# jzbontar/mc-cnn

Measured on AMD Instinct MI355X. Metric: Mega-pixel-disparities/sec (cost-vol+CBCA+SGM) + end-to-end disp ms/pair, higher is better.
Workload: dtype f32; 1 GPU; KITTI 2012 fast, 370x1226 disp_max=228; H=370, W=1226, disp_max=228, feature_channels=64, params=kitti_fast, parallelism=one pair per GPU

## Files before the change

### mc-cnn_amd/csrc/api.hip

```cpp
#include "launchers.h"

using namespace mc;

#define MC_REQUIRE_DIRECTION(name, direction) MC_REQUIRE((direction) == -1 || (direction) == 1, name ": direction must be -1 or 1")

struct PlanArea { size_t off, bytes; };
static PlanArea plan_area(int D, int H, int W) { return {align_up(cbca_scratch_bytes(H, W), 256), cbca_plan_bytes(D, H, W)}; }

extern "C" {

int mc_version(void) { return MC_ABI_VERSION; }
const char *mc_last_error(void) { return last_error(); }

int mc_fill_nan(float *p, int64_t n, void *stream)
{
	MC_REQUIRE(p || n == 0, "mc_fill_nan: null pointer");
	MC_REQUIRE(n >= 0, "mc_fill_nan: negative size");
	return fill_nan(p, n, as_stream(stream));
}

int mc_stereo_join(const float *featL, const float *featR, float *volL, float *volR, int C, int D, int H, int W, void *stream)
{
	MC_REQUIRE(featL && featR && volL && volR, "mc_stereo_join: null pointer");
	MC_REQUIRE(dims_ok(D, H, W) && C >= 1, "mc_stereo_join: bad dims C=%d D=%d H=%d W=%d", C, D, H, W);
// ... 240 lines not shown

size_t mc_sgm2_tmp_bytes(int H, int W, int D)
{
	(void)D;
	if (H < 1 || W < 1) return 0;
	return sgm_maps_bytes(H, W);
}

int mc_sgm2(const float *x0, const float *x1, const float *in_hwd, float *out_hwd, void *tmp, size_t tmp_bytes, int H, int W,
            int D, float pi1, float pi2, float tau_so, float alpha1, float sgm_q1, float sgm_q2, int direction, void *stream)
{
	MC_REQUIRE(x0 && x1 && in_hwd && out_hwd && tmp, "mc_sgm2: null pointer");
	MC_REQUIRE(dims_ok(D, H, W), "mc_sgm2: bad dims");
	MC_REQUIRE(D <= MC_SGM_MAX_D, "mc_sgm2: D=%d exceeds %d", D, MC_SGM_MAX_D);
	MC_REQUIRE_DIRECTION("mc_sgm2", direction);
	MC_REQUIRE(tmp_bytes >= sgm_maps_bytes(H, W), "mc_sgm2: tmp holds %zu bytes, needs %zu", tmp_bytes, sgm_maps_bytes(H, W));
	MC_REQUIRE(in_hwd != out_hwd, "mc_sgm2: input and output must differ");
	hipStream_t st = as_stream(stream);
	int rc = sgm_prep(x0, x1, tmp, H, W, tau_so, st);
	if (rc) return rc;
	const float *Cv[2] = {in_hwd, in_hwd};
	float *outv[2] = {out_hwd, out_hwd};
	const int dirv[2] = {direction, direction};
	return sgm_sweeps(Cv, outv, nullptr, nullptr, dirv, 1, H, W, D, D, tmp, pi1, pi2, alpha1, sgm_q1, sgm_q2, false, 0u, false, st);
}

int mc_dhw_to_hwd(const float *in, float *out, int D, int H, int W, void *stream)
{
	MC_REQUIRE(in && out && in != out, "mc_dhw_to_hwd: bad pointers");
	MC_REQUIRE(dims_ok(D, H, W), "mc_dhw_to_hwd: bad dims");
	return transpose(in, out, D, (int64_t)H * W, (int64_t)H * W, D, 1.0f, as_stream(stream));
}

int mc_hwd_to_dhw(const float *in, float *out, int D, int H, int W, float scale_, void *stream)
{
	MC_REQUIRE(in && out && in != out, "mc_hwd_to_dhw: bad pointers");
	MC_REQUIRE(dims_ok(D, H, W), "mc_hwd_to_dhw: bad dims");
	return transpose(in, out, (int64_t)H * W, D, D, (int64_t)H * W, scale_, as_stream(stream));
}

int mc_scale(const float *in, float *out, int64_t n, float s, void *stream)
{
	MC_REQUIRE((in && out) || n == 0, "mc_scale: null pointer");
	MC_REQUIRE(n >= 0, "mc_scale: negative size");
	return scale(in, out, n, s, as_stream(stream));
}

int mc_argmin(const float *vol, float *disp, int D, int H, int W, void *stream)
{
	MC_REQUIRE(vol && disp, "mc_argmin: null pointer");
	MC_REQUIRE(dims_ok(D, H, W), "mc_argmin: bad dims");
	return argmin_dhw(vol, disp, D, H, W, 0, as_stream(stream));
}

int mc_spatial_argmin(const float *vol, float *out, int D, int H, int W, void *stream)
{
	MC_REQUIRE(vol && out, "mc_spatial_argmin: null pointer");
	MC_REQUIRE(dims_ok(D, H, W), "mc_spatial_argmin: bad dims");
	return argmin_dhw(vol, out, D, H, W, 1, as_stream(stream));
}

int mc_outlier_detection(const float *d0, const float *d1, float *outlier, int H, int W, int disp_max, void *stream)
{
	MC_REQUIRE(d0 && d1 && outlier, "mc_outlier_detection: null pointer");
	MC_REQUIRE(dims_ok(1, H, W) && disp_max >= 0, "mc_outlier_detection: bad dims");
	return outlier_detection(d0, d1, outlier, H, W, disp_max, as_stream(stream));
}

int mc_interpolate_occlusion(const float *d0, const float *outlier, float *out, int H, int W, void *stream)
{
	MC_REQUIRE(d0 && outlier && out && out != d0, "mc_interpolate_occlusion: bad pointers");
	MC_REQUIRE(dims_ok(1, H, W), "mc_interpolate_occlusion: bad dims");
	return interpolate_occlusion(d0, outlier, out, H, W, as_stream(stream));
}

int mc_interpolate_mismatch(const float *d0, const float *outlier, float *out, int H, int W, void *stream)
{
	MC_REQUIRE(d0 && outlier && out && out != d0, "mc_interpolate_mismatch: bad pointers");
	MC_REQUIRE(dims_ok(1, H, W), "mc_interpolate_mismatch: bad dims");
	return interpolate_mismatch(d0, outlier, out, H, W, as_stream(stream));
}

int mc_subpixel_enchancement(const float *d0, const float *vol, float *out, int D, int H, int W, void *stream)
{
	MC_REQUIRE(d0 && vol && out, "mc_subpixel_enchancement: null pointer");
	MC_REQUIRE(dims_ok(D, H, W), "mc_subpixel_enchancement: bad dims");
	return subpixel(d0, vol, out, D, H, W, (int64_t)H * W, 1, as_stream(stream));
}

int mc_median2d(const float *img, float *out, int H, int W, int kernel_size, void *stream)
{
	MC_REQUIRE(img && out && img != out, "mc_median2d: bad pointers");
	MC_REQUIRE(dims_ok(1, H, W), "mc_median2d: bad dims");
	MC_REQUIRE(kernel_size % 2 == 1 && kernel_size >= 1 && kernel_size <= 11,
	           "mc_median2d: kernel_size must be odd and <= 11 (adcensus.cu:1601-1602)");
	return median2d(img, out, H, W, kernel_size, as_stream(stream));
}

int mc_mean2d(const float *img, const float *kernel, float *out, int H, int W, int ks, float alpha2, void *stream)
{
	MC_REQUIRE(img && kernel && out && img != out, "mc_mean2d: bad pointers");
	MC_REQUIRE(dims_ok(1, H, W), "mc_mean2d: bad dims");
	MC_REQUIRE(ks % 2 == 1 && ks >= 1, "mc_mean2d: kernel size must be odd (adcensus.cu:1269)");
	return mean2d(img, kernel, out, H, W, ks, alpha2, as_stream(stream));
}

int mc_gaussian_host(double sigma, float *host_kernel, int capacity)
{
	MC_REQUIRE(sigma > 0, "mc_gaussian_host: sigma must be > 0");
	const int ks = gaussian_ks(sigma);
	if (host_kernel) {
		MC_REQUIRE(capacity >= ks * ks, "mc_gaussian_host: capacity %d < %d", capacity, ks * ks);
		gaussian_fill(sigma, host_kernel);
	}
	return ks;
}

int mc_normalize_forward(const float *in, float *norm, float *out, int N, int C, int H, int W, void *stream)
{
	MC_REQUIRE(in && out, "mc_normalize_forward: null pointer");
	MC_REQUIRE(N >= 1 && C >= 1 && dims_ok(1, H, W), "mc_normalize_forward: bad dims");
	return normalize_forward(in, norm, out, N, C, H, W, as_stream(stream));
}

size_t mc_predict_workspace_bytes(const mc_params *p, int C, int D, int H, int W)
{
	(void)C;
	if (!p || !dims_ok(D, H, W) || !(p->blur_sigma > 0)) return 0;
	return make_plan(p, D, H, W).total;
}

int mc_predict(const mc_params *p, const float *x0, const float *x1, const float *featL, const float *featR, int C,
               const float *rawL, const float *rawR, int D, int H, int W, void *workspace, size_t workspace_bytes,
               float *volL_out, float *volR_out, float *dispL0_out, float *dispR0_out, float *disp_out, void *stream)
{
	StageTimer tm;
	return predict_impl(p, x0, x1, featL, featR, C, rawL, rawR, D, H, W, workspace, workspace_bytes, volL_out, volR_out,
	                    dispL0_out, dispR0_out, disp_out, as_stream(stream), tm);
}

int mc_predict_timed(const mc_params *p, const float *x0, const float *x1, const float *featL, const float *featR, int C,
                     const float *rawL, const float *rawR, int D, int H, int W, void *workspace, size_t workspace_bytes,
                     float *disp_out, void *stream, float *stage_ms)
{
	StageTimer tm;
	tm.on = stage_ms != nullptr;
	tm.st = as_stream(stream);
	const int rc = predict_impl(p, x0, x1, featL, featR, C, rawL, rawR, D, H, W, workspace, workspace_bytes, nullptr, nullptr,
	                            nullptr, nullptr, disp_out, tm.st, tm);
	if (stage_ms) tm.collect(stage_ms);
	return rc;
}

}
```

### mc-cnn_amd/csrc/launchers.h

```cpp
#pragma once
#include "cbca_common.h"

#include <vector>

namespace mc {

int fill_nan(float *p, int64_t n, hipStream_t st);
int scale(const float *in, float *out, int64_t n, float s, hipStream_t st);
int transpose(const float *in, float *out, int64_t R, int64_t Cn, int64_t ldin, int64_t ldout, float s, hipStream_t st, int nt = -1);
int fix_border(float *vol, int D, int H, int W, int n, int direction, hipStream_t st);
int argmin_dhw(const float *vol, float *out, int D, int H, int W, int base1, hipStream_t st);
int outlier_detection(const float *d0, const float *d1, float *outlier, int H, int W, int disp_max, hipStream_t st);
constexpr int MC_MIS_MASK_MAX_PIXELS = 524288;
int interpolate_occlusion(const float *d0, const float *outlier, float *out, int H, int W, hipStream_t st, unsigned *mask = nullptr);
int interpolate_mismatch(const float *d0, const float *outlier, float *out, int H, int W, hipStream_t st, const unsigned *mask = nullptr);
int subpixel(const float *d0, const float *vol, float *out, int D, int H, int W, int64_t sd, int64_t sp, hipStream_t st);
int median2d(const float *img, float *out, int H, int W, int k, hipStream_t st);
int mean2d(const float *img, const float *kernel, float *out, int H, int W, int ks, float alpha2, hipStream_t st);
int normalize_forward(const float *in, float *norm, float *out, int N, int C, int H, int W, hipStream_t st);

int stereo_join_dhw(const float *fL, const float *fR, float *volL, float *volR, int C, int D, int H, int W, hipStream_t st);
int stereo_join_hwd(const float *fL, const float *fR, float *volL, float *volR, int C, int D, int ds, int H, int W, int n, hipStream_t st);
int ad_tiled(const float *x0, const float *x1, float *vol, int D, int H, int W, int direction, hipStream_t st);
size_t census_scratch_bytes(int Cimg, int H, int W);
int census_sig(const float *x0, const float *x1, float *vol, void *scratch, int Cimg, int D, int H, int W, int direction, hipStream_t st);

int cross(const float *img, float *arms, int H, int W, int L1, float tau1, hipStream_t st);
int cbca(const float *x0c, const float *x1c, const float *vin, float *vout, int D, int H, int W, int direction, hipStream_t st);
size_t cbca_scratch_bytes(int H, int W);
int cbca_pack(const float *x0c, const float *x1c, void *scratch, int H, int W, hipStream_t st);
int cbca_if_overflow(const float *x0c, const float *x1c, const void *packed, const float *vin, float *vout, int D, int H, int W, int direction, hipStream_t st);
int cbca_strips(const void *packed, const float *vin, float *vout, int D, int H, int W, int direction, int route,
                hipStream_t st, const CbcaCfg &cfg = CbcaCfg());
bool packed_dims_ok(int H, int W);
int cbca_by_arms(const void *packed, const float *vin, float *vout, int D, int H, int W, int direction, int max_arm, hipStream_t st,
                 const CbcaCfg &cfg = CbcaCfg());

size_t cbca_plan_bytes(int D, int H, int W);
int cbca_tiles(const void *packed, const float *vin, float *vout, int D, int H, int W, int direction, int arm_class, int route,
               hipStream_t st, const CbcaCfg &cfg = CbcaCfg());

int cbca_lean_rows(int D, int H, int W, int rb, bool two_pass);
size_t cbca_lean2x_bytes(int D, int H, int W);
bool cbca_lean_fits(int D, int H, int W, size_t plan_bytes, bool two_pass = false, int rb = 0);
int cbca_classify(const void *packed, void *plan, size_t plan_bytes, int D, int H, int W, int direction, int route, int rb, int cap_limit,
                  hipStream_t st, bool two_pass = false, float cost_limit = 0);
int cbca_lean2x(const void *packed, const void *plan, size_t plan_bytes, const float *vin, float *vout, int D, int H, int W, int direction,
                int route, hipStream_t st, const CbcaCfg &cfg);
int cbca_lean(const void *packed, const void *plan, size_t plan_bytes, const float *vin, float *vout, int D, int H, int W, int direction,
              int route, hipStream_t st, const CbcaCfg &cfg);

size_t conv3x3_workspace_bytes(int Cin, int Cout);
int conv3x3(const float *in, const float *w, const float *bias, float *out, int N, int Cin, int Cout, int H, int W, int relu, void *workspace, hipStream_t st);

size_t fc_workspace_bytes(int C, int n_hidden, int H, int W);
int fc_stack(const float *featL, const float *featR, int C, int H, int W, int D, const float *const *weights,
             const float *const *biases, int n_layers, float *volL, float *volR, void *workspace, hipStream_t st);

size_t sgm_maps_bytes(int H, int W);
int sgm_prep(const float *x0, const float *x1, void *maps, int H, int W, float tau_so, hipStream_t st);
int sgm_contract_violations(const float *vol, int H, int W, int D, unsigned *count, hipStream_t st);
int sgm_sweeps(const float *const C[2], float *const out[2], float *const out2[2], float *const disp[2],
               const int direction[2], int nvol, int H, int W, int D, int ds, const void *maps, float pi1, float pi2,
               float alpha1, float q1, float q2, bool fused, unsigned drop_final, bool tri, hipStream_t st);

static inline int gaussian_ks(double sigma) { return 2 * (int)ceil(sigma * 3) + 1; }
void gaussian_fill(double sigma, float *k);

struct Plan {
	int Dp;
	size_t cplan_bytes;
	size_t total;
	void *maps, *packed;
	float *x0c, *x1c, *img[6], *gk;
	float *bufA[2], *bufB[2], *bufC[2];
	void *cplan[2];
};
Plan make_plan(const mc_params *p, int D, int H, int W, void *base = nullptr);

struct StageTimer {
	bool on = false;
	hipStream_t st;
	std::vector<hipEvent_t> ev;
	std::vector<int> tag;
	void mark(int stage);
	void collect(float out[MC_N_STAGES]);
};
int predict_impl(const mc_params *p, const float *x0, const float *x1, const float *featL, const float *featR, int C,
                 const float *rawL, const float *rawR, int D, int H, int W, void *workspace, size_t workspace_bytes,
                 float *volL_out, float *volR_out, float *dispL0_out, float *dispR0_out, float *disp_out, hipStream_t st,
                 StageTimer &tm);

}
```

### mc-cnn_amd/csrc/predict.hip

```cpp
#include "launchers.h"

#include <map>
#include <mutex>
#include <utility>

namespace mc {

void gaussian_fill(double sigma, float *k)
{
	const int ks = gaussian_ks(sigma), kr = ks / 2;
	for (int i = 1; i <= ks; ++i) {
		for (int j = 1; j <= ks; ++j) {
			const double y = (i - 1) - kr;
			const double x = (j - 1) - kr;
			k[(size_t)(i - 1) * ks + (j - 1)] = (float)exp(-(x * x + y * y) / (2 * sigma * sigma));
		}
	}
}
static int gaussian_cached(double sigma, const float *&out)
{
	static std::mutex mu;
	static std::map<std::pair<int, double>, const float *> cache;
	int dev = 0;
	hipError_t e = hipGetDevice(&dev);
	if (e != hipSuccess) {
		set_error("gaussian: hipGetDevice: %s", hipGetErrorString(e));
		return (int)e;
	}
	std::lock_guard<std::mutex> lk(mu);
	auto it = cache.find({dev, sigma});
	if (it != cache.end()) { out = it->second; return 0; }
	const int ks = gaussian_ks(sigma);
	std::vector<float> k((size_t)ks * ks);
	gaussian_fill(sigma, k.data());
	float *dk = nullptr;
	e = hipMalloc((void **)&dk, k.size() * sizeof(float));
	if (e == hipSuccess) e = hipMemcpy(dk, k.data(), k.size() * sizeof(float), hipMemcpyHostToDevice);
	if (e != hipSuccess) {
		set_error("gaussian: device table of %zu floats: %s", k.size(), hipGetErrorString(e));
		if (dk) (void)hipFree(dk);
		return (int)e;
	}
	out = cache[{dev, sigma}] = dk;
	return 0;
}

struct StageCounts { int cbca1, sgm, cbca2; bool active_after; };
static StageCounts stage_counts(const mc_params *p)
{
	StageCounts c;
	bool sm_active = p->sm_terminate != MC_SM_CNN;
	c.cbca1 = (sm_active && p->sm_skip != MC_SKIP_CBCA) ? p->cbca_i1 : 0;
	sm_active = sm_active && p->sm_terminate != MC_SM_CBCA1;
	c.sgm = (sm_active && p->sm_skip != MC_SKIP_SGM) ? p->sgm_i : 0;
	sm_active = sm_active && p->sm_terminate != MC_SM_SGM;
	c.cbca2 = (sm_active && p->sm_skip != MC_SKIP_CBCA) ? p->cbca_i2 : 0;
	sm_active = sm_active && p->sm_terminate != MC_SM_CBCA2;
	c.active_after = sm_active;
	return c;
}

Plan make_plan(const mc_params *p, int D, int H, int W, void *base)
{
	Plan pl;
	pl.Dp = (D + 3) / 4 * 4;
	const size_t HW = (size_t)H * W;
	const size_t vol = align_up((size_t)pl.Dp * HW * sizeof(float), 256), img = align_up(HW * sizeof(float), 256);
	const int ks = gaussian_ks(p->blur_sigma);
	const StageCounts sc = stage_counts(p);
	pl.cplan_bytes = (sc.cbca1 + sc.cbca2 >= 2 && p->L1 - 1 <= 13) ? align_up(cbca_plan_bytes(D, H, W), 256) : 0;
	const int nplan = (p->left_only && !p->lr_check) ? 1 : 2;

	size_t off = 0;
	auto take = [&](size_t bytes) { off += bytes; return base ? (char *)base + (off - bytes) : nullptr; };
	pl.maps = take(align_up(sgm_maps_bytes(H, W), 256));
	pl.x0c = (float *)take(align_up(8 * HW * sizeof(float), 256));
	pl.x1c = base ? pl.x0c + 4 * HW : nullptr;
	pl.packed = take(cbca_scratch_bytes(H, W));
	for (float **buf : {pl.bufA, pl.bufB, pl.bufC})
		for (int v = 0; v < 2; ++v) buf[v] = (float *)take(vol);
	for (float *&im : pl.img) im = (float *)take(img);
	pl.gk = (float *)take(align_up((size_t)ks * ks * sizeof(float), 256));
	for (int v = 0; v < 2; ++v) pl.cplan[v] = (pl.cplan_bytes && v < nplan) ? take(pl.cplan_bytes) : nullptr;
	pl.total = off;
	return pl;
}

void StageTimer::mark(int stage)
{
	if (!on) return;
	hipEvent_t e;
	(void)hipEventCreate(&e);
	(void)hipEventRecord(e, st);
	ev.push_back(e);
	tag.push_back(stage);
}
void StageTimer::collect(float out[MC_N_STAGES])
{
	for (int i = 0; i < MC_N_STAGES; ++i) out[i] = 0;
	if (!on || ev.empty()) return;
	(void)hipEventSynchronize(ev.back());
	for (size_t i = 1; i < ev.size(); ++i) {
		float ms = 0;
		(void)hipEventElapsedTime(&ms, ev[i - 1], ev[i]);
		if (tag[i] >= 0 && tag[i] < MC_N_STAGES) out[tag[i]] += ms;
	}
	for (auto e : ev) (void)hipEventDestroy(e);
	ev.clear();
}

int predict_impl(const mc_params *p, const float *x0, const float *x1, const float *featL, const float *featR, int C,
                 const float *rawL, const float *rawR, int D, int H, int W, void *workspace, size_t workspace_bytes,
                 float *volL_out, float *volR_out, float *dispL0_out, float *dispR0_out, float *disp_out, hipStream_t st,
                 StageTimer &tm)
{
	MC_REQUIRE(p && x0 && x1 && disp_out && workspace, "mc_predict: null argument");
	MC_REQUIRE(dims_ok(D, H, W), "mc_predict: bad dims D=%d H=%d W=%d", D, H, W);
	MC_REQUIRE(D <= MC_SGM_MAX_D, "mc_predict: D=%d exceeds %d", D, MC_SGM_MAX_D);
	MC_REQUIRE((featL && featR && C >= 1) || (rawL && rawR), "mc_predict: need features or raw volumes");
	MC_REQUIRE(p->cbca_i1 >= 0 && p->cbca_i2 >= 0 && p->sgm_i >= 0, "mc_predict: negative iteration count");
	MC_REQUIRE(p->median_k % 2 == 1 && p->median_k <= 11, "mc_predict: median_k must be odd and <= 11");
	MC_REQUIRE(p->blur_sigma > 0, "mc_predict: blur_sigma must be > 0");
	MC_REQUIRE(p->sm_terminate >= 0 && p->sm_terminate <= MC_SM_BILATERAL && p->sm_skip >= 0 && p->sm_skip <= MC_SKIP_BILATERAL,
	           "mc_predict: bad sm_terminate / sm_skip");
	const bool from_feat = featL != nullptr;
	if (from_feat) MC_REQUIRE(p->border_n >= 0 && p->border_n < W, "mc_predict: border_n=%d out of range", p->border_n);
	if (from_feat) MC_REQUIRE(C <= MC_JOIN_MAX_C, "mc_predict: C=%d exceeds %d (adcensus.cu:1460)", C, MC_JOIN_MAX_C);
	const Plan pl = make_plan(p, D, H, W, workspace);
	MC_REQUIRE(workspace_bytes >= pl.total, "mc_predict: workspace %zu < %zu bytes", workspace_bytes, pl.total);
	MC_REQUIRE((uintptr_t)workspace % 256 == 0, "mc_predict: workspace must be 256-byte aligned");

	const int64_t HW = (int64_t)H * W;
	const int64_t V = (int64_t)D * HW;
	int cplan_passes[2] = {0, 0};
	bool cplan_listed[2] = {false, false};
	int rc;
#define RUN(call) do { rc = (call); if (rc) return rc; } while (0)

	const int direction[2] = {-1, 1};
	const StageCounts sc = stage_counts(p);
	const int n_cbca1 = sc.cbca1, n_sgm = sc.sgm, n_cbca2 = sc.cbca2;
	bool sm_active = sc.active_after;
	const bool use_cbca = (n_cbca1 + n_cbca2) > 0;
	tm.mark(-1);

	if (n_sgm > 0) RUN(sgm_prep(x0, x1, pl.maps, H, W, p->tau_so, st));
	if (use_cbca) {
		RUN(cross(x0, pl.x0c, H, W, p->L1, p->tau1, st));
		RUN(cross(x1, pl.x1c, H, W, p->L1, p->tau1, st));
		RUN(cbca_pack(pl.x0c, pl.x1c, pl.packed, H, W, st));
	}
	const int cbca_cap = p->L1 - 1;
	tm.mark(MC_STAGE_PREP);

	const int ds = pl.Dp;
	const float *cur[2];
	auto other = [&](int v) -> float * { return cur[v] == pl.bufA[v] ? pl.bufB[v] : pl.bufA[v]; };
	bool hwd;
	const int nvol = (p->left_only && !p->lr_check && !volR_out && !dispR0_out) ? 1 : 2;
	auto cbca_iterations = [&](int n) -> int {
		const bool packed_ok = cbca_cap <= 254 && packed_dims_ok(H, W);
		for (int v = 0; v < nvol; ++v) {
			const bool planned = packed_ok && pl.cplan[v] && cbca_cap > 4 && cbca_cap <= 13 && cbca_lean_fits(D, H, W, pl.cplan_bytes, true);
			if (planned && n > 0 && !cplan_listed[v]) {
				const int rc1 = cbca_classify(pl.packed, pl.cplan[v], pl.cplan_bytes, D, H, W, direction[v], CR_STRIP, 0, 0, st, true);
				if (rc1) return rc1;
				cplan_listed[v] = true;
			}
			for (int i = 0; i < n;) {
				float *dst = other(v);
				CbcaCfg cfg;
				cfg.plan = pl.cplan[v];
				cfg.plan_bytes = pl.cplan_bytes;
				cfg.planned = planned;
				const bool two = planned && i + 1 < n;
				cfg.lean = cfg.lean_two_pass = two;
				float *mid = two ? pl.bufC[v] : dst;
				for (int half = 0; half < (two ? 2 : 1); ++half) {
					cfg.plan_mode = pl.cplan[v] ? (cplan_passes[v]++ == 0 ? 1 : 2) : 0;
					const float *src = half == 0 ? cur[v] : mid;
					float *to = (two && half == 0) ? mid : dst;
					const int rc2 = packed_ok ? cbca_by_arms(pl.packed, src, to, D, H, W, direction[v], cbca_cap, st, cfg)
					                          : cbca(pl.x0c, pl.x1c, src, to, D, H, W, direction[v], st);
					if (rc2) return rc2;
				}
				if (two) {
					const int rc3 = cbca_lean2x(pl.packed, pl.cplan[v], pl.cplan_bytes, cur[v], dst, D, H, W, direction[v], CR_STRIP, st, cfg);
					if (rc3) return rc3;
				}
				cur[v] = dst;
				i += two ? 2 : 1;
			}
		}
		return 0;
	};
	const bool join_fits = (int64_t)W * ((D + 3) / 4 * 4) * 4 < ((int64_t)1 << 31) && ((int64_t)(C + 64) * HW + W) * 4 < ((int64_t)1 << 31);
	bool nan_triangle = false;
	if (from_feat && n_cbca1 == 0 && n_sgm > 0 && join_fits) {
		RUN(stereo_join_hwd(featL, featR, pl.bufA[0], pl.bufA[1], C, D, ds, H, W, p->border_n, st));
		cur[0] = pl.bufA[0]; cur[1] = pl.bufA[1];
		hwd = true;
		nan_triangle = true;
		tm.mark(MC_STAGE_JOIN);
	} else {
		if (from_feat) {
			RUN(fill_nan(pl.bufA[0], V, st));
			RUN(fill_nan(pl.bufA[1], V, st));
			RUN(stereo_join_dhw(featL, featR, pl.bufA[0], pl.bufA[1], C, D, H, W, st));
			RUN(fix_border(pl.bufA[0], D, H, W, p->border_n, -1, st));
			RUN(fix_border(pl.bufA[1], D, H, W, p->border_n, 1, st));
			cur[0] = pl.bufA[0]; cur[1] = pl.bufA[1];
		} else {
			cur[0] = rawL; cur[1] = rawR;
		}
		hwd = false;
		tm.mark(MC_STAGE_JOIN);
		RUN(cbca_iterations(n_cbca1));
		tm.mark(MC_STAGE_CBCA);
	}

	float *dispv[2] = {pl.img[0], pl.img[1]};
	bool have_disp = false;
	if (n_sgm > 0) {
		if (!hwd) {
			for (int v = 0; v < nvol; ++v) {
				float *dst = other(v);
				RUN(transpose(cur[v], dst, D, HW, HW, ds, 1.0f, st));
				cur[v] = dst;
			}
			hwd = true;
			tm.mark(MC_STAGE_LAYOUT);
		}
		for (int it = 0; it < n_sgm; ++it) {
			const float *Cv[2] = {cur[0], cur[1]};
			float *outv[2] = {other(0), other(1)};
			const bool am = (it == n_sgm - 1) && n_cbca2 == 0;
			const unsigned drop_final = (am && nvol == 2 && !volR_out) ? 2u : 0u;
			RUN(sgm_sweeps(Cv, outv, pl.bufC, am ? dispv : nullptr, direction, nvol, H, W, D, ds, pl.maps, p->pi1, p->pi2, p->alpha1,
			               p->sgm_q1, p->sgm_q2, true, drop_final, nan_triangle, st));
			have_disp = am;
			cur[0] = outv[0]; cur[1] = outv[1];
		}
		tm.mark(MC_STAGE_SGM);
		if (n_cbca2 > 0) {
			for (int v = 0; v < nvol; ++v) {
				float *dst = other(v);
				RUN(transpose(cur[v], dst, HW, D, ds, HW, 1.0f, st));
				cur[v] = dst;
			}
			hwd = false;
			tm.mark(MC_STAGE_LAYOUT);
		}
	}
	if (!hwd) {
		RUN(cbca_iterations(n_cbca2));
		tm.mark(MC_STAGE_CBCA);
	}

	MC_REQUIRE(have_disp || !hwd, "mc_predict: an (H,W,D) volume without its arg-min");
	if (!have_disp) {
		for (int v = 0; v < nvol; ++v) RUN(argmin_dhw(cur[v], dispv[v], D, H, W, 0, st));
	}
	float *vout[2] = {volL_out, volR_out};
	for (int v = 0; v < nvol; ++v) {
		if (!vout[v]) continue;
		if (hwd) RUN(transpose(cur[v], vout[v], HW, D, ds, HW, 1.0f, st));
		else RUN(scale(cur[v], vout[v], V, 1.0f, st));
	}
	if (dispL0_out) RUN(scale(dispv[0], dispL0_out, HW, 1.0f, st));
	if (dispR0_out) RUN(scale(dispv[1], dispR0_out, HW, 1.0f, st));
	tm.mark(MC_STAGE_ARGMIN);

	float *d = dispv[0];
	float *outl = pl.img[4];
	int nfree = 0;
	float *freeimg[3] = {pl.img[2], pl.img[3], pl.img[5]};
	auto next = [&]() -> float * {
		float *r = freeimg[nfree % 3];
		if (r == d) r = freeimg[++nfree % 3];
		++nfree;
		return r;
	};
	auto stage = [&](int skip, int terminate, auto &&run) -> int {
		if (sm_active && p->sm_skip != skip) {
			float *o = next();
			if (const int rc1 = run(o)) return rc1;
			d = o;
		}
		sm_active = sm_active && p->sm_terminate != terminate;
		return 0;
	};
	if (p->lr_check) {
		RUN(outlier_detection(d, dispv[1], outl, H, W, D, st));
		const unsigned *mis_mask = nullptr;
		RUN(stage(MC_SKIP_OCCLUSION, MC_SM_OCCLUSION, [&](float *o) {
			unsigned *m = HW <= MC_MIS_MASK_MAX_PIXELS ? (unsigned *)pl.x0c : nullptr;
			mis_mask = m;
			return interpolate_occlusion(d, outl, o, H, W, st, m);
		}));
		RUN(stage(MC_SKIP_OCCLUSION, MC_SM_MISMATCH, [&](float *o) { return interpolate_mismatch(d, outl, o, H, W, st, mis_mask); }));
	}
	RUN(stage(MC_SKIP_SUBPIXEL, MC_SM_SUBPIXEL, [&](float *o) {
		return hwd ? subpixel(d, cur[0], o, D, H, W, 1, ds, st) : subpixel(d, cur[0], o, D, H, W, HW, 1, st);
	}));
	RUN(stage(MC_SKIP_MEDIAN, MC_SM_MEDIAN, [&](float *o) { return median2d(d, o, H, W, p->median_k, st); }));
	if (sm_active && p->sm_skip != MC_SKIP_BILATERAL) {
		const float *gk = nullptr;
		RUN(gaussian_cached(p->blur_sigma, gk));
		RUN(mean2d(d, gk, disp_out, H, W, gaussian_ks(p->blur_sigma), p->blur_t, st));
	} else {
		RUN(scale(d, disp_out, HW, 1.0f, st));
	}
	tm.mark(MC_STAGE_POST);
#undef RUN
	return 0;
}

}
```

### mc-cnn_amd/csrc/stereo_join.hip

```cpp
#include "launchers.h"
#include <type_traits>

namespace mc {

constexpr int JD_PX = 64, JD_D = 32, JD_CK = 16, JD_RW = JD_PX + JD_D;

__global__ void __launch_bounds__(256) join_dhw_kernel(const float *__restrict__ fL, const float *__restrict__ fR,
                                                       float *__restrict__ volL, float *__restrict__ volR, int C, int D, int H, int W)
{
	__shared__ float Ls[JD_CK][JD_PX];
	__shared__ float Rs[JD_CK][JD_RW];
	const int tid = threadIdx.x, xi = tid & 63, dg = tid >> 6;
	const int x0 = blockIdx.x * JD_PX, y = blockIdx.y, d0 = blockIdx.z * JD_D;
	const int64_t HW = (int64_t)H * W;
	const float *__restrict__ rowL = fL + (int64_t)y * W;
	const float *__restrict__ rowR = fR + (int64_t)y * W;
	const int r0 = x0 - d0 - (JD_D - 1);
	float sum[8];
#pragma unroll
	for (int k = 0; k < 8; ++k) sum[k] = 0.0f;
	for (int c0 = 0; c0 < C; c0 += JD_CK) {
		__syncthreads();
		for (int e = tid; e < JD_CK * JD_PX; e += 256) {
			const int c = e / JD_PX, i = e % JD_PX;
// ... 117 lines not shown
				__builtin_amdgcn_raw_buffer_store_b32(__float_as_uint(qok ? acc[i] : NANV), rowL,
				                                      ok ? (unsigned)(off + mo * (ds + 1)) * 4u : 0x80000000u, 0, 0);
			}
		}
#pragma unroll
		for (int i = 0; i < 16; ++i) {
			const int m = (i & 3) + 8 * (i >> 2) + 4 * kh;
			Tw[m * 33 + nl] = acc[i];
		}
		{
			const int mL = nl;
			const bool pin = p0 + mL < W;
			const int offR = (q0 + kh) * ds + mL - kh + 32 * J;
#pragma unroll
			for (int i = 0; i < 16; ++i) {
				const int n = 2 * i + kh;
				const int xr = q0 + n;
				const int d = mL - n + 32 * J;
				const bool ok = xr >= 0 && xr < W && d >= 0 && d < D;
				const float v = Tw[mL * 33 + n];
				__builtin_amdgcn_raw_buffer_store_b32(__float_as_uint(pin ? v : NANV), rowR,
				                                      ok ? (unsigned)(offR + 2 * i * (ds - 1)) * 4u : 0x80000000u, 0, 0);
			}
		}
#pragma unroll
		for (int kk = 0; kk < KSTEPS; ++kk) bcur[kk] = bnxt[kk];
	}
}

#define MC_JOIN_STORE_AUX 2

template <int KSTEPS, int SIDE, int NT>
__device__ __forceinline__ void join_owner_tiles(const float *__restrict__ fL, const float *__restrict__ fR, float *__restrict__ vol,
                                                 int C, int D, int ds, int H, int W, int y, int tile0, float *__restrict__ rings)
{
	const int lane = threadIdx.x & 63;
	const int nl = lane & 31, kh = lane >> 5;
	const int64_t HW = (int64_t)H * W;
	const unsigned feat_bytes = (unsigned)(((int64_t)(C - 1) * HW + W) * 4);
	const __amdgpu_buffer_rsrc_t rA = __builtin_amdgcn_make_buffer_rsrc((void *)(fL + (int64_t)y * W), 0, feat_bytes, 0x00020000);
	const __amdgpu_buffer_rsrc_t rB = __builtin_amdgcn_make_buffer_rsrc((void *)(fR + (int64_t)y * W), 0, feat_bytes, 0x00020000);
	const unsigned pair_bytes = (unsigned)(2 * HW * 4);
	const unsigned OOBF = 0x80000000u;
	const float NANV = __builtin_nanf("");
	auto load_tile = [&](float (&v)[KSTEPS], const __amdgpu_buffer_rsrc_t &r, int p0, bool negate) {
		const int px = p0 + nl;
		const unsigned vo = (px >= 0 && px < W) ? (unsigned)((int64_t)kh * HW + px) * 4u : OOBF;
#pragma unroll
		for (int kk = 0; kk < KSTEPS; ++kk) {
			const float t = __uint_as_float(__builtin_amdgcn_raw_buffer_load_b32(r, vo + (unsigned)kk * pair_bytes, 0, 0));
			v[kk] = negate ? -t : t;
		}
	};
	auto load_partner = [&](float (&v)[KSTEPS], int T) { load_tile(v, SIDE == 0 ? rB : rA, 32 * T, false); };
	float own[NT][KSTEPS], pa[KSTEPS], pb[KSTEPS];
#pragma unroll
	for (int t = 0; t < NT; ++t) load_tile(own[t], SIDE == 0 ? rA : rB, 32 * (tile0 + t), true);
	const int nJ = (D + 30) / 32 + 1;
	const int nsteps = nJ + NT - 1;
	auto partner_of = [&](int s) { return SIDE == 0 ? tile0 + NT - 1 - s : tile0 + s; };
	load_partner(pa, partner_of(0));

	const int wbase = 4 * kh - nl;
	const int wrow = SIDE == 0 ? 4 * kh * 64 : nl * 64;

	const int fp = lane & 7;
	const int row_floats = W * ds;
	const __amdgpu_buffer_rsrc_t rrow = __builtin_amdgcn_make_buffer_rsrc((void *)(vol + (int64_t)y * row_floats), 0, row_floats * 4, 0x00020000);
	const int row_mis = (int)(((int64_t)y * row_floats) & 31);
	int fd0[NT][4];
	unsigned fgo[NT][4];
#pragma unroll
	for (int t = 0; t < NT; ++t) {
#pragma unroll
		for (int pass = 0; pass < 4; ++pass) {
			const int px = 32 * (tile0 + t) + pass * 8 + (lane >> 3);
			const int fo = pass * 8 + (lane >> 3);
			const int a_o = (row_mis + px * ds) & 31;
			const int c_o = SIDE == 0 ? fo : 31 - fo;
			const int kl = ((c_o + a_o - 63 + 64) >> 5) - 2 + 1;
			fd0[t][pass] = 32 * kl - a_o + 4 * fp;
			fgo[t][pass] = px < W ? (unsigned)(px * ds) * 4u : OOBF;
		}
	}
	auto tile_product = [&](int t, const float (&part)[KSTEPS], int p0, floatx16 &acc) {
#pragma unroll
		for (int i = 0; i < 16; ++i) acc[i] = 0.0f;
		const bool any_in = SIDE == 0 ? (p0 + 31 >= 0) : (p0 < W);
		if (any_in) {
#pragma unroll
			for (int kk = 0; kk < KSTEPS; ++kk)
				acc = SIDE == 0 ? __builtin_amdgcn_mfma_f32_32x32x2f32(own[t][kk], part[kk], acc, 0, 0, 0)
				                : __builtin_amdgcn_mfma_f32_32x32x2f32(part[kk], own[t][kk], acc, 0, 0, 0);
		}
	};
	auto tile_store = [&](int t, int J, int p0, const floatx16 &acc) {
		float *__restrict__ ring = rings + t * (32 * 64);
		const int jbit = (J & 1) << 5;
		const bool interior = J >= 1 && 32 * J + 31 < D && (SIDE == 0 ? p0 >= 0 : p0 + 31 < W);
		if (interior) {
#pragma unroll
			for (int i = 0; i < 16; ++i) {
				const int mc = (i & 3) + 8 * (i >> 2);
				ring[wrow + (SIDE == 0 ? mc * 64 : 0) + (((wbase + mc) & 63) ^ jbit)] = acc[i];
			}
		} else {
#pragma unroll
			for (int i = 0; i < 16; ++i) {
				const int mc = (i & 3) + 8 * (i >> 2);
				const int d = wbase + mc + 32 * J;
				const int po = SIDE == 0 ? p0 + nl : p0 + mc + 4 * kh;
				const bool pin = SIDE == 0 ? po >= 0 : po < W;
				if (d >= 0 && d < D) ring[wrow + (SIDE == 0 ? mc * 64 : 0) + (((wbase + mc) & 63) ^ jbit)] = pin ? acc[i] : NANV;
			}
		}
		const bool last = J + 1 == nJ;
#pragma unroll
		for (int pass = 0; pass < 4; ++pass) {
			const int d0 = fd0[t][pass] + 32 * J;
			const int fro = (pass * 8 + (lane >> 3)) * 64;
			const float4 v = *(const float4 *)(ring + fro + (d0 & 63));
			__builtin_amdgcn_raw_buffer_store_b128((cb_u4_t){__float_as_uint(v.x), __float_as_uint(v.y), __float_as_uint(v.z), __float_as_uint(v.w)},
			                                       rrow, ((unsigned)d0 < (unsigned)ds) ? fgo[t][pass] + (unsigned)d0 * 4u : OOBF, 0, MC_JOIN_STORE_AUX);
			if (last) {
				const int d1 = d0 + 32;
				const float4 u = *(const float4 *)(ring + fro + (d1 & 63));
				__builtin_amdgcn_raw_buffer_store_b128((cb_u4_t){__float_as_uint(u.x), __float_as_uint(u.y), __float_as_uint(u.z), __float_as_uint(u.w)},
				                                       rrow, ((unsigned)d1 < (unsigned)ds) ? fgo[t][pass] + (unsigned)d1 * 4u : OOBF, 0, MC_JOIN_STORE_AUX);
			}
		}
	};
	auto do_step = [&](int s, const float (&part)[KSTEPS]) {
		const int T = partner_of(s);
		floatx16 acc[NT];
#pragma unroll
		for (int t = 0; t < NT; ++t) {
			const int J = SIDE == 0 ? tile0 + t - T : T - tile0 - t;
			if (J >= 0 && J < nJ) { tile_product(t, part, 32 * T, acc[0]); tile_store(t, J, 32 * T, acc[0]); }
		}
	};
	for (int s = 0; s < nsteps; s += 2) {
		load_partner(pb, partner_of(s + 1));
		do_step(s, pa);
		load_partner(pa, partner_of(s + 2));
		if (s + 1 < nsteps) do_step(s + 1, pb);
	}
}

#define MC_JOIN_NT 2
#define MC_JOIN_WPB 4
template <int KSTEPS, int NT = MC_JOIN_NT>
__global__ void __launch_bounds__(64 * MC_JOIN_WPB) join_owner_kernel(const float *__restrict__ fL, const float *__restrict__ fR,
                                                         float *__restrict__ volL, float *__restrict__ volR, int C, int D, int ds,
                                                         int H, int W, int pairs_per_row)
{
	__shared__ __attribute__((aligned(16))) float rings[MC_JOIN_WPB][NT * 32 * 64];
	const int wid = __builtin_amdgcn_readfirstlane(threadIdx.x >> 6);
	const int b = blockIdx.x;
	const int xcd = b & 7, k = b >> 3;
	const int blocks_per_row = (2 * pairs_per_row + MC_JOIN_WPB - 1) / MC_JOIN_WPB;
	const int y = (k / blocks_per_row) * 8 + xcd;
	const int w = (k % blocks_per_row) * MC_JOIN_WPB + wid;
	if (y >= H || w >= 2 * pairs_per_row) return;
	if (w < pairs_per_row) join_owner_tiles<KSTEPS, 0, NT>(fL, fR, volL, C, D, ds, H, W, y, NT * w, rings[wid]);
	else join_owner_tiles<KSTEPS, 1, NT>(fL, fR, volR, C, D, ds, H, W, y, NT * (w - pairs_per_row), rings[wid]);
}

__global__ void __launch_bounds__(256) fix_border_hwd_kernel(float *__restrict__ volL, float *__restrict__ volR, int D, int ds, int H,
                                                             int W, int n)
{
	const int lane = threadIdx.x & 63;
	int64_t w = ((int64_t)blockIdx.x * blockDim.x + threadIdx.x) >> 6;
	const int64_t per = (int64_t)H * n;
	if (w >= 2 * per) return;
	const bool right = w >= per;
	if (right) w -= per;
	float *vol = right ? volR : volL;
	const int y = (int)(w / n), i = (int)(w % n) + 1;
	const int dst = right ? i - 1 : W - i;
	const int src = right ? n : W - (n + 1);
	const float *s = vol + ((int64_t)y * W + src) * ds;
	float *t = vol + ((int64_t)y * W + dst) * ds;
	for (int d = lane; d < D; d += 64) t[d] = s[d];
}

int stereo_join_hwd(const float *fL, const float *fR, float *volL, float *volR, int C, int D, int ds, int H, int W, int n,
                    hipStream_t st)
{
	const int rows8 = (H + 7) / 8;
	const int ks = (C + 1) / 2;
	const dim3 block(256);
	MC_REQUIRE(ds % 4 == 0 && (uintptr_t)volL % 16 == 0 && (uintptr_t)volR % 16 == 0,
	           "stereo_join_hwd: the volumes must be 16-byte aligned with a pixel stride ds %% 4 == 0 (ds = %d)", ds);
	const char *what = "stereo_join_hwd";
	if (ks <= 32) {
		const int tiles_own = ((W + 31) / 32 + MC_JOIN_NT - 1) / MC_JOIN_NT;
		const dim3 grid_o((unsigned)(rows8 * ((2 * tiles_own + MC_JOIN_WPB - 1) / MC_JOIN_WPB) * 8)), block_o(64 * MC_JOIN_WPB);
		if (ks <= 8) hipLaunchKernelGGL((join_owner_kernel<8>), grid_o, block_o, 0, st, fL, fR, volL, volR, C, D, ds, H, W, tiles_own);
		else if (ks <= 16) hipLaunchKernelGGL((join_owner_kernel<16>), grid_o, block_o, 0, st, fL, fR, volL, volR, C, D, ds, H, W, tiles_own);
		else hipLaunchKernelGGL((join_owner_kernel<32>), grid_o, block_o, 0, st, fL, fR, volL, volR, C, D, ds, H, W, tiles_own);
		what = "stereo_join_hwd (owner tiles)";
	} else {
		const int tiles = (W + D - 1 + 31) / 32;
		const int blocks_per_row = (tiles + 3) / 4;
		const dim3 grid((unsigned)(rows8 * blocks_per_row * 8));
		if (ks <= 56) hipLaunchKernelGGL((join_mfma_kernel<56>), grid, block, 0, st, fL, fR, volL, volR, C, D, ds, H, W, tiles);
		else hipLaunchKernelGGL((join_mfma_kernel<64>), grid, block, 0, st, fL, fR, volL, volR, C, D, ds, H, W, tiles);
	}
	const int rc = check_launch(what);
	if (rc || n <= 0) return rc;
	hipLaunchKernelGGL(fix_border_hwd_kernel, dim3(cdiv((int64_t)2 * H * n * 64, 256)), block, 0, st, volL, volR, D, ds, H, W, n);
	return check_launch("fix_border_hwd");
}

__global__ void __launch_bounds__(256) census_sig_kernel(const float *__restrict__ img, uint32_t *__restrict__ sig,
                                                         uint32_t *__restrict__ mask, int Cimg, int H, int W)
{
	const int64_t id = (int64_t)blockIdx.x * blockDim.x + threadIdx.x;
	const int64_t HW = (int64_t)H * W;
	if (id >= (int64_t)Cimg * HW) return;
	const int c = (int)(id / HW);
	const int64_t pix = id - c * HW;
	const int x = (int)(pix % W), y = (int)(pix / W);
	const float *__restrict__ im = img + c * HW;
	const float p = im[pix];
	uint32_t s[3] = {0, 0, 0}, m[3] = {0, 0, 0};
	int t = 0;
	for (int yy = y - 4; yy <= y + 4; yy++) {
		for (int xx = x - 4; xx <= x + 4; xx++, t++) {
			if (0 <= xx && xx < W && 0 <= yy && yy < H) {
				m[t >> 5] |= 1u << (t & 31);
				if (im[(int64_t)yy * W + xx] < p) s[t >> 5] |= 1u << (t & 31);
			}
		}
	}
	uint32_t *so = sig + id * 3;
	so[0] = s[0]; so[1] = s[1]; so[2] = s[2];
	if (c == 0) {
		uint32_t *mo = mask + pix * 3;
		mo[0] = m[0]; mo[1] = m[1]; mo[2] = m[2];
	}
}

__global__ void __launch_bounds__(256) census_cost_kernel(const uint32_t *__restrict__ sig0, const uint32_t *__restrict__ sig1,
                                                          const uint32_t *__restrict__ mask, float *__restrict__ out, int Cimg, int D,
                                                          int H, int W, int direction)
{
	const int x = blockIdx.x * 256 + threadIdx.x;
	const int y = blockIdx.y;
	const int d = blockIdx.z * direction;
	if (x >= W) return;
	const int64_t HW = (int64_t)H * W;
	const int64_t pix = (int64_t)y * W + x;
	float dist;
	if (0 <= x + d && x + d < W) {
		const uint32_t *m0 = mask + pix * 3, *m1 = mask + (pix + d) * 3;
		const uint32_t v0 = m0[0] & m1[0], v1 = m0[1] & m1[1], v2 = m0[2] & m1[2];
		const int oob = 81 - (__popc(v0) + __popc(v1) + __popc(v2));
		dist = 0;
		for (int c = 0; c < Cimg; c++) {
			const uint32_t *a = sig0 + (c * HW + pix) * 3, *b = sig1 + (c * HW + pix + d) * 3;
			const int diff = __popc((a[0] ^ b[0]) & v0) + __popc((a[1] ^ b[1]) & v1) + __popc((a[2] ^ b[2]) & v2);
			dist += (float)(oob + diff);
		}
		dist /= (float)Cimg;
	} else {
		dist = __builtin_nanf("");
	}
	out[(int64_t)blockIdx.z * HW + pix] = dist;
}

size_t census_scratch_bytes(int Cimg, int H, int W)
{
	return (((size_t)2 * Cimg + 1) * H * W * 3 * sizeof(uint32_t) + 255) & ~(size_t)255;
}

int census_sig(const float *x0, const float *x1, float *vol, void *scratch, int Cimg, int D, int H, int W, int direction,
               hipStream_t st)
{
	const int64_t HW = (int64_t)H * W;
	uint32_t *s0 = (uint32_t *)scratch, *s1 = s0 + (size_t)Cimg * HW * 3, *mk = s1 + (size_t)Cimg * HW * 3;
	hipLaunchKernelGGL(census_sig_kernel, dim3(cdiv((int64_t)Cimg * HW, 256)), dim3(256), 0, st, x0, s0, mk, Cimg, H, W);
	hipLaunchKernelGGL(census_sig_kernel, dim3(cdiv((int64_t)Cimg * HW, 256)), dim3(256), 0, st, x1, s1, mk, Cimg, H, W);
	hipLaunchKernelGGL(census_cost_kernel, dim3(cdiv(W, 256), H, D), dim3(256), 0, st, s0, s1, mk, vol, Cimg, D, H, W, direction);
	return check_launch("census");
}

__global__ void __launch_bounds__(256) ad_tile_kernel(const float *__restrict__ x0, const float *__restrict__ x1, float *__restrict__ out,
                                                      int D, int H, int W, int direction)
{
	constexpr int TY = 16, TX = 64, R = 4, TS = TX + 2 * R + 1;
	__shared__ float A[(TY + 2 * R) * TS];
	const int bx = blockIdx.x * TX, by = blockIdx.y * TY;
	const int d = blockIdx.z * direction;
	const float NANV = __builtin_nanf("");
	for (int i = threadIdx.x; i < (TY + 2 * R) * (TX + 2 * R); i += 256) {
		const int ty = i / (TX + 2 * R), tx = i - ty * (TX + 2 * R);
		const int yy = by + ty - R, xx = bx + tx - R;
		float v = NANV;
		if (0 <= xx && xx < W && 0 <= xx + d && xx + d < W && 0 <= yy && yy < H) {
			const int64_t ind = (int64_t)yy * W + xx;
			v = fabsf(x0[ind] - x1[ind + d]);
		}
		A[ty * TS + tx] = v;
	}
	__syncthreads();
	const int lx = threadIdx.x & 63, wv = threadIdx.x >> 6;
	const int x = bx + lx;
	if (x >= W) return;
	const int64_t HW = (int64_t)H * W;
	for (int r = wv; r < TY; r += 4) {
		const int y = by + r;
		if (y >= H) break;
		float dist;
		if (0 <= x + d && x + d < W) {
			int cnt = 0;
			dist = 0;
			const float *base = A + r * TS + lx;
#pragma unroll
			for (int j = 0; j < 2 * R + 1; ++j) {
#pragma unroll
				for (int k = 0; k < 2 * R + 1; ++k) {
					const float v = base[j * TS + k];
					const bool ok = v == v;
					dist += ok ? v : -0.0f;
					cnt += ok ? 1 : 0;
				}
			}
			dist /= (float)cnt;
		} else {
			dist = NANV;
		}
		out[(int64_t)blockIdx.z * HW + (int64_t)y * W + x] = dist;
	}
}

int ad_tiled(const float *x0, const float *x1, float *vol, int D, int H, int W, int direction, hipStream_t st)
{
	hipLaunchKernelGGL(ad_tile_kernel, dim3(cdiv(W, 64), cdiv(H, 16), D), dim3(256), 0, st, x0, x1, vol, D, H, W, direction);
	return check_launch("ad");
}

}
```

Measured before the change: 83100 MPix-disp/s.

## Run right-view join and SGM on a side stream overlapping the left view

Splits the stereo join into separate left and right launches and runs the right view's join, SGM iterations and output copies on a cached side stream, joined back with events before post-processing. This is meant to overlap the two views' work and hide the join/SGM serialization and per-kernel tail effects on one stream. By default the side lane waits for the left join to finish first (staggered). It adds stream/event management, a per-stream lock and cache, and a fallback to a single lane when several callers share the device. The two views may contend for the same compute units, so the overlap may not help.

```diff
diff --git a/mc-cnn_amd/csrc/api.hip b/mc-cnn_amd/csrc/api.hip
--- a/mc-cnn_amd/csrc/api.hip
+++ b/mc-cnn_amd/csrc/api.hip
@@ -416,4 +416,18 @@
 	return rc;
 }
 
-}
+#pragma GCC visibility push(default)
+int mc_test_predict_lanes(int set) { return predict_lanes(set); }
+
+int mc_test_stereo_join_hwd(const float *featL, const float *featR, float *volL, float *volR, int C, int D, int ds, int H, int W, int border_n,
+                            int sides, void *stream)
+{
+	MC_REQUIRE(featL && featR && volL && volR, "mc_test_stereo_join_hwd: null pointer");
+	MC_REQUIRE(dims_ok(D, H, W) && C >= 1 && C <= MC_JOIN_MAX_C && ds >= D && border_n >= 0 && border_n < W, "mc_test_stereo_join_hwd: bad dims");
+	const int64_t HW = (int64_t)H * W;
+	MC_REQUIRE((int64_t)W * ds * 4 < ((int64_t)1 << 31) && ((int64_t)(C + 64) * HW + W) * 4 < ((int64_t)1 << 31), "mc_test_stereo_join_hwd: too large");
+	return stereo_join_hwd(featL, featR, volL, volR, C, D, ds, H, W, border_n, as_stream(stream), sides);
+}
+#pragma GCC visibility pop
+
+}
diff --git a/mc-cnn_amd/csrc/launchers.h b/mc-cnn_amd/csrc/launchers.h
--- a/mc-cnn_amd/csrc/launchers.h
+++ b/mc-cnn_amd/csrc/launchers.h
@@ -1,6 +1,7 @@
 #pragma once
 #include "cbca_common.h"
 
+#include <mutex>
 #include <vector>
 
 namespace mc {
@@ -20,7 +21,8 @@
 int normalize_forward(const float *in, float *norm, float *out, int N, int C, int H, int W, hipStream_t st);
 
 int stereo_join_dhw(const float *fL, const float *fR, float *volL, float *volR, int C, int D, int H, int W, hipStream_t st);
-int stereo_join_hwd(const float *fL, const float *fR, float *volL, float *volR, int C, int D, int ds, int H, int W, int n, hipStream_t st);
+int stereo_join_hwd(const float *fL, const float *fR, float *volL, float *volR, int C, int D, int ds, int H, int W, int n, hipStream_t st,
+                    int sides = 3);
 int ad_tiled(const float *x0, const float *x1, float *vol, int D, int H, int W, int direction, hipStream_t st);
 size_t census_scratch_bytes(int Cimg, int H, int W);
 int census_sig(const float *x0, const float *x1, float *vol, void *scratch, int Cimg, int D, int H, int W, int direction, hipStream_t st);
@@ -78,6 +80,14 @@
 };
 Plan make_plan(const mc_params *p, int D, int H, int W, void *base = nullptr);
 
+int parse_predict_lanes(const char *s);
+int predict_lanes(int set = -1, bool *is_forced = nullptr);
+struct Lanes {
+	hipStream_t side = nullptr;
+	hipEvent_t fork = nullptr, join_left = nullptr, right_done = nullptr;
+	std::mutex mu;
+};
+
 struct StageTimer {
 	bool on = false;
 	hipStream_t st;
diff --git a/mc-cnn_amd/csrc/predict.hip b/mc-cnn_amd/csrc/predict.hip
--- a/mc-cnn_amd/csrc/predict.hip
+++ b/mc-cnn_amd/csrc/predict.hip
@@ -1,5 +1,6 @@
 #include "launchers.h"
 
+#include <atomic>
 #include <map>
 #include <mutex>
 #include <utility>
@@ -44,6 +45,81 @@
 	out = cache[{dev, sigma}] = dk;
 	return 0;
 }
+
+int parse_predict_lanes(const char *s) { return (s && s[0] == '1' && s[1] == '\0') ? 1 : 2; }
+int predict_lanes(int set, bool *is_forced)
+{
+	static const int from_env = parse_predict_lanes(getenv("MC_PREDICT_LANES"));
+	static std::atomic<int> forced{0};
+	if (set >= 0 && set <= 2) forced.store(set);
+	const int f = forced.load();
+	if (is_forced) *is_forced = f != 0;
+	return f ? f : from_env;
+}
+
+#define MC_HIP(call, what) do { const hipError_t e_ = (call); if (e_ != hipSuccess) { set_error("mc_predict: %s: %s", what, hipGetErrorString(e_)); return (int)e_; } } while (0)
+
+static int lanes_cached(hipStream_t st, bool solo_only, Lanes *&out, std::unique_lock<std::mutex> &held)
+{
+	static std::mutex mu;
+	static auto &cache = *new std::map<std::pair<int, hipStream_t>, Lanes *>;
+	static auto &first_caller = *new std::map<int, hipStream_t>;
+	static auto &many_callers = *new std::map<int, bool>;
+	int dev = 0;
+	MC_HIP(hipGetDevice(&dev), "hipGetDevice");
+	std::lock_guard<std::mutex> lk(mu);
+	out = nullptr;
+	if (solo_only) {
+		auto fc = first_caller.find(dev);
+		if (fc == first_caller.end()) first_caller[dev] = st;
+		else if (fc->second != st) many_callers[dev] = true;
+		if (many_callers[dev]) {
+			for (auto it = cache.begin(); it != cache.end();) {
+				Lanes *l = it->second;
+				if (it->first.first != dev || !l->mu.try_lock()) { ++it; continue; }
+				(void)hipStreamDestroy(l->side);
+				for (hipEvent_t ev : {l->fork, l->join_left, l->right_done}) (void)hipEventDestroy(ev);
+				l->mu.unlock();
+				delete l;
+				it = cache.erase(it);
+			}
+			return 0;
+		}
+	}
+	auto it = cache.find({dev, st});
+	if (it == cache.end()) {
+		Lanes *l = new Lanes;
+		hipError_t e = hipStreamCreateWithFlags(&l->side, hipStreamNonBlocking);
+		hipEvent_t *const evs[3] = {&l->fork, &l->join_left, &l->right_done};
+		for (int i = 0; i < 3 && e == hipSuccess; ++i) e = hipEventCreateWithFlags(evs[i], hipEventDisableTiming);
+		if (e != hipSuccess) {
+			set_error("mc_predict: side stream and events: %s", hipGetErrorString(e));
+			for (hipEvent_t *ev : evs) if (*ev) (void)hipEventDestroy(*ev);
+			if (l->side) (void)hipStreamDestroy(l->side);
+			delete l;
+			return (int)e;
+		}
+		it = cache.emplace(std::make_pair(dev, st), l).first;
+	}
+	out = it->second;
+	held = std::unique_lock<std::mutex>(out->mu);
+	return 0;
+}
+
+struct LaneJoin {
+	hipStream_t st = nullptr;
+	Lanes *ln = nullptr;
+	bool armed = false;
+	int join()
+	{
+		if (!armed) return 0;
+		armed = false;
+		MC_HIP(hipEventRecord(ln->right_done, ln->side), "hipEventRecord (right lane done)");
+		MC_HIP(hipStreamWaitEvent(st, ln->right_done, 0), "hipStreamWaitEvent (right lane done)");
+		return 0;
+	}
+	~LaneJoin() { (void)join(); }
+};
 
 struct StageCounts { int cbca1, sgm, cbca2; bool active_after; };
 static StageCounts stage_counts(const mc_params *p)
@@ -196,11 +272,53 @@
 	};
 	const bool join_fits = (int64_t)W * ((D + 3) / 4 * 4) * 4 < ((int64_t)1 << 31) && ((int64_t)(C + 64) * HW + W) * 4 < ((int64_t)1 << 31);
 	bool nan_triangle = false;
+	float *dispv[2] = {pl.img[0], pl.img[1]};
+	bool have_disp = false;
+	auto sgm_iterations = [&](int v0, int nv, hipStream_t s) -> int {
+		for (int it = 0; it < n_sgm; ++it) {
+			const float *Cv[2];
+			float *outv[2], *scratch[2], *dv[2];
+			int dir[2];
+			for (int k = 0; k < nv; ++k) {
+				Cv[k] = cur[v0 + k]; outv[k] = other(v0 + k); scratch[k] = pl.bufC[v0 + k]; dv[k] = dispv[v0 + k]; dir[k] = direction[v0 + k];
+			}
+			const bool am = (it == n_sgm - 1) && n_cbca2 == 0;
+			const bool has_right = v0 + nv == 2;
+			const unsigned drop_final = (am && has_right && !volR_out) ? 1u << (1 - v0) : 0u;
+			const int rc1 = sgm_sweeps(Cv, outv, scratch, am ? dv : nullptr, dir, nv, H, W, D, ds, pl.maps, p->pi1, p->pi2, p->alpha1,
+			                           p->sgm_q1, p->sgm_q2, true, drop_final, nan_triangle, s);
+			if (rc1) return rc1;
+			have_disp = am;
+			for (int k = 0; k < nv; ++k) cur[v0 + k] = outv[k];
+		}
+		return 0;
+	};
+	std::unique_lock<std::mutex> lane_lock;
+	LaneJoin lane_b;
 	if (from_feat && n_cbca1 == 0 && n_sgm > 0 && join_fits) {
-		RUN(stereo_join_hwd(featL, featR, pl.bufA[0], pl.bufA[1], C, D, ds, H, W, p->border_n, st));
+		bool forced = false;
+		const bool two_lanes = nvol == 2 && n_cbca2 == 0 && C <= 64 && !tm.on && predict_lanes(-1, &forced) == 2;
 		cur[0] = pl.bufA[0]; cur[1] = pl.bufA[1];
 		hwd = true;
 		nan_triangle = true;
+		Lanes *ln = nullptr;
+		if (two_lanes) RUN(lanes_cached(st, !forced, ln, lane_lock));
+		if (ln) {
+			MC_HIP(hipEventRecord(ln->fork, st), "hipEventRecord (fork)");
+			RUN(stereo_join_hwd(featL, featR, pl.bufA[0], pl.bufA[1], C, D, ds, H, W, p->border_n, st, 1));
+			MC_HIP(hipEventRecord(ln->join_left, st), "hipEventRecord (left join)");
+			lane_b.st = st; lane_b.ln = ln; lane_b.armed = true;
+			MC_HIP(hipStreamWaitEvent(ln->side, ln->fork, 0), "hipStreamWaitEvent (fork)");
+#ifndef MC_LANES_NO_STAGGER
+			MC_HIP(hipStreamWaitEvent(ln->side, ln->join_left, 0), "hipStreamWaitEvent (left join)");
+#endif
+			RUN(stereo_join_hwd(featL, featR, pl.bufA[0], pl.bufA[1], C, D, ds, H, W, p->border_n, ln->side, 2));
+			RUN(sgm_iterations(1, 1, ln->side));
+			if (volR_out) RUN(transpose(cur[1], volR_out, HW, D, ds, HW, 1.0f, ln->side));
+			if (dispR0_out) RUN(scale(dispv[1], dispR0_out, HW, 1.0f, ln->side));
+		} else {
+			RUN(stereo_join_hwd(featL, featR, pl.bufA[0], pl.bufA[1], C, D, ds, H, W, p->border_n, st));
+		}
 		tm.mark(MC_STAGE_JOIN);
 	} else {
 		if (from_feat) {
@@ -219,8 +337,7 @@
 		tm.mark(MC_STAGE_CBCA);
 	}
 
-	float *dispv[2] = {pl.img[0], pl.img[1]};
-	bool have_disp = false;
+	const int nmain = lane_b.armed ? 1 : nvol;
 	if (n_sgm > 0) {
 		if (!hwd) {
 			for (int v = 0; v < nvol; ++v) {
@@ -231,16 +348,7 @@
 			hwd = true;
 			tm.mark(MC_STAGE_LAYOUT);
 		}
-		for (int it = 0; it < n_sgm; ++it) {
-			const float *Cv[2] = {cur[0], cur[1]};
-			float *outv[2] = {other(0), other(1)};
-			const bool am = (it == n_sgm - 1) && n_cbca2 == 0;
-			const unsigned drop_final = (am && nvol == 2 && !volR_out) ? 2u : 0u;
-			RUN(sgm_sweeps(Cv, outv, pl.bufC, am ? dispv : nullptr, direction, nvol, H, W, D, ds, pl.maps, p->pi1, p->pi2, p->alpha1,
-			               p->sgm_q1, p->sgm_q2, true, drop_final, nan_triangle, st));
-			have_disp = am;
-			cur[0] = outv[0]; cur[1] = outv[1];
-		}
+		RUN(sgm_iterations(0, nmain, st));
 		tm.mark(MC_STAGE_SGM);
 		if (n_cbca2 > 0) {
 			for (int v = 0; v < nvol; ++v) {
@@ -262,14 +370,16 @@
 		for (int v = 0; v < nvol; ++v) RUN(argmin_dhw(cur[v], dispv[v], D, H, W, 0, st));
 	}
 	float *vout[2] = {volL_out, volR_out};
-	for (int v = 0; v < nvol; ++v) {
+	for (int v = 0; v < nmain; ++v) {
 		if (!vout[v]) continue;
 		if (hwd) RUN(transpose(cur[v], vout[v], HW, D, ds, HW, 1.0f, st));
 		else RUN(scale(cur[v], vout[v], V, 1.0f, st));
 	}
 	if (dispL0_out) RUN(scale(dispv[0], dispL0_out, HW, 1.0f, st));
-	if (dispR0_out) RUN(scale(dispv[1], dispR0_out, HW, 1.0f, st));
+	if (dispR0_out && nmain == nvol) RUN(scale(dispv[1], dispR0_out, HW, 1.0f, st));
 	tm.mark(MC_STAGE_ARGMIN);
+	RUN(lane_b.join());
+	if (lane_lock.owns_lock()) lane_lock.unlock();
 
 	float *d = dispv[0];
 	float *outl = pl.img[4];
@@ -313,6 +423,7 @@
 	}
 	tm.mark(MC_STAGE_POST);
 #undef RUN
+#undef MC_HIP
 	return 0;
 }
 
diff --git a/mc-cnn_amd/csrc/stereo_join.hip b/mc-cnn_amd/csrc/stereo_join.hip
--- a/mc-cnn_amd/csrc/stereo_join.hip
+++ b/mc-cnn_amd/csrc/stereo_join.hip
@@ -293,29 +293,31 @@
 template <int KSTEPS, int NT = MC_JOIN_NT>
 __global__ void __launch_bounds__(64 * MC_JOIN_WPB) join_owner_kernel(const float *__restrict__ fL, const float *__restrict__ fR,
                                                          float *__restrict__ volL, float *__restrict__ volR, int C, int D, int ds,
-                                                         int H, int W, int pairs_per_row)
+                                                         int H, int W, int pairs_per_row, int sides)
 {
 	__shared__ __attribute__((aligned(16))) float rings[MC_JOIN_WPB][NT * 32 * 64];
 	const int wid = __builtin_amdgcn_readfirstlane(threadIdx.x >> 6);
 	const int b = blockIdx.x;
 	const int xcd = b & 7, k = b >> 3;
-	const int blocks_per_row = (2 * pairs_per_row + MC_JOIN_WPB - 1) / MC_JOIN_WPB;
+	const int row_waves = sides == 3 ? 2 * pairs_per_row : pairs_per_row;
+	const int blocks_per_row = (row_waves + MC_JOIN_WPB - 1) / MC_JOIN_WPB;
 	const int y = (k / blocks_per_row) * 8 + xcd;
-	const int w = (k % blocks_per_row) * MC_JOIN_WPB + wid;
-	if (y >= H || w >= 2 * pairs_per_row) return;
+	const int w0 = (k % blocks_per_row) * MC_JOIN_WPB + wid;
+	if (y >= H || w0 >= row_waves) return;
+	const int w = sides == 2 ? w0 + pairs_per_row : w0;
 	if (w < pairs_per_row) join_owner_tiles<KSTEPS, 0, NT>(fL, fR, volL, C, D, ds, H, W, y, NT * w, rings[wid]);
 	else join_owner_tiles<KSTEPS, 1, NT>(fL, fR, volR, C, D, ds, H, W, y, NT * (w - pairs_per_row), rings[wid]);
 }
 
 __global__ void __launch_bounds__(256) fix_border_hwd_kernel(float *__restrict__ volL, float *__restrict__ volR, int D, int ds, int H,
-                                                             int W, int n)
+                                                             int W, int n, int sides)
 {
 	const int lane = threadIdx.x & 63;
 	int64_t w = ((int64_t)blockIdx.x * blockDim.x + threadIdx.x) >> 6;
 	const int64_t per = (int64_t)H * n;
-	if (w >= 2 * per) return;
-	const bool right = w >= per;
-	if (right) w -= per;
+	if (w >= (sides == 3 ? 2 * per : per)) return;
+	const bool right = sides == 2 || w >= per;
+	if (w >= per) w -= per;
 	float *vol = right ? volR : volL;
 	const int y = (int)(w / n), i = (int)(w % n) + 1;
 	const int dst = right ? i - 1 : W - i;
@@ -326,20 +328,22 @@
 }
 
 int stereo_join_hwd(const float *fL, const float *fR, float *volL, float *volR, int C, int D, int ds, int H, int W, int n,
-                    hipStream_t st)
+                    hipStream_t st, int sides)
 {
 	const int rows8 = (H + 7) / 8;
 	const int ks = (C + 1) / 2;
 	const dim3 block(256);
 	MC_REQUIRE(ds % 4 == 0 && (uintptr_t)volL % 16 == 0 && (uintptr_t)volR % 16 == 0,
 	           "stereo_join_hwd: the volumes must be 16-byte aligned with a pixel stride ds %% 4 == 0 (ds = %d)", ds);
+	MC_REQUIRE(sides >= 1 && sides <= 3 && (sides == 3 || ks <= 32), "stereo_join_hwd: sides=%d (C = %d)", sides, C);
+	const int nside = sides == 3 ? 2 : 1;
 	const char *what = "stereo_join_hwd";
 	if (ks <= 32) {
 		const int tiles_own = ((W + 31) / 32 + MC_JOIN_NT - 1) / MC_JOIN_NT;
-		const dim3 grid_o((unsigned)(rows8 * ((2 * tiles_own + MC_JOIN_WPB - 1) / MC_JOIN_WPB) * 8)), block_o(64 * MC_JOIN_WPB);
-		if (ks <= 8) hipLaunchKernelGGL((join_owner_kernel<8>), grid_o, block_o, 0, st, fL, fR, volL, volR, C, D, ds, H, W, tiles_own);
-		else if (ks <= 16) hipLaunchKernelGGL((join_owner_kernel<16>), grid_o, block_o, 0, st, fL, fR, volL, volR, C, D, ds, H, W, tiles_own);
-		else hipLaunchKernelGGL((join_owner_kernel<32>), grid_o, block_o, 0, st, fL, fR, volL, volR, C, D, ds, H, W, tiles_own);
+		const dim3 grid_o((unsigned)(rows8 * ((nside * tiles_own + MC_JOIN_WPB - 1) / MC_JOIN_WPB) * 8)), block_o(64 * MC_JOIN_WPB);
+		if (ks <= 8) hipLaunchKernelGGL((join_owner_kernel<8>), grid_o, block_o, 0, st, fL, fR, volL, volR, C, D, ds, H, W, tiles_own, sides);
+		else if (ks <= 16) hipLaunchKernelGGL((join_owner_kernel<16>), grid_o, block_o, 0, st, fL, fR, volL, volR, C, D, ds, H, W, tiles_own, sides);
+		else hipLaunchKernelGGL((join_owner_kernel<32>), grid_o, block_o, 0, st, fL, fR, volL, volR, C, D, ds, H, W, tiles_own, sides);
 		what = "stereo_join_hwd (owner tiles)";
 	} else {
 		const int tiles = (W + D - 1 + 31) / 32;
@@ -350,7 +354,7 @@
 	}
 	const int rc = check_launch(what);
 	if (rc || n <= 0) return rc;
-	hipLaunchKernelGGL(fix_border_hwd_kernel, dim3(cdiv((int64_t)2 * H * n * 64, 256)), block, 0, st, volL, volR, D, ds, H, W, n);
+	hipLaunchKernelGGL(fix_border_hwd_kernel, dim3(cdiv((int64_t)nside * H * n * 64, 256)), block, 0, st, volL, volR, D, ds, H, W, n, sides);
 	return check_launch("fix_border_hwd");
 }
 
```

Measured after the change: 85260 MPix-disp/s (median of 6 runs). +2.6%, better.
